# andrew-sha/CUDAFluidSimulator

Measured on AMD Instinct MI355X. Metric: particle-steps/sec (first 41 of the 100 steps of -m time), higher is better.
Workload: dtype f32

## Files before the change

cudafluidsimulator_amd/csrc/sph_api.hip:

```cpp
#include "sph_handle.h"

#include <algorithm>
#include <cmath>
#include <cstdio>
#include <cstdlib>
#include <cstring>
#include <vector>

using namespace sph_host;

namespace {

thread_local std::string g_create_error;

float force_cut2(float h) {
    float h2 = h * h;
    float x = h2;
    for (int k = 0; k < 64; ++k) {
        float nx = std::nextafterf(x, INFINITY);
        if (sqrtf(nx) <= h) x = nx;
        else break;
    }
    return x;
}

Knobs read_knobs() {
    Knobs k;
    if (const char *e = getenv("SPH_SLIM_DIV")) k.slimDiv = atoi(e);
    if (const char *e = getenv("SPH_PIPELINE")) k.pipeline = atoi(e) != 0;
    if (const char *e = getenv("SPH_MASK_POOL_WORDS")) k.maskPoolSet = true, k.maskPoolQuads = strtoull(e, nullptr, 10) / 4;
    if (const char *e = getenv("SPH_ZERO_PAIR_FILTER")) k.zeroPairFilter = atoi(e) != 0;
    if (const char *e = getenv("SPH_PREWARM_COPIES")) k.prewarmCopies = atoi(e);
    if (const char *e = getenv("SPH_TILE_CHUNK")) k.tileChunk = atoi(e);
    if (const char *e = getenv("SPH_XCD_ROTATE")) k.xcdRotate = atoi(e);
    if (const char *e = getenv("SPH_STEP_TRACE")) k.stepTrace = atoi(e) != 0;
    if (const char *e = getenv("SPH_READBACK_SDMA")) k.readbackSdma = atoi(e) != 0;
    return k;
}

void fill_params(sph_handle *h) {
    const SphSettings &s = h->settings;
    DevParams &P = h->P;
    P.h = s.h;
    P.h2 = s.h * s.h;
    P.vcoef = s.v_kernel_coeff;
    P.dcoef = s.d_kernel_coeff;
    P.boxDim = s.boxDim;
    P.boxHi = s.boxDim - s.h;
    P.dt = s.timestep;
    P.cut2 = force_cut2(s.h);
    P.D = (int)s.numCellsPerDim;
    P.morton = h->opt.key_order == SPH_KEY_MORTON ? 1 : 0;
    {
        SphSettings ref{};
        sph_default_settings(&ref, s.numParticles, s.randomInit);
        P.slimDiv = (s.h == ref.h && s.v_kernel_coeff == ref.v_kernel_coeff && s.d_kernel_coeff == ref.d_kernel_coeff) ? 1 : 0;
        if (h->knobs.slimDiv == 0) P.slimDiv = 0;
    }
    if (P.morton) {
        int b = 0;
        while ((1 << b) < P.D) ++b;
        P.numCells = 1 << (3 * b);
    } else {
        P.numCells = P.D * P.D * P.D;
    }
}

int init_positions_reference(const SphSettings &s, float *pos) {
    int n = s.numParticles;
    if (s.randomInit) {
        srand(1);
        for (int i = 0; i < n; i++) {
            float x = rand() / (float)RAND_MAX * (s.boxDim - 2.f) + 1.f;
            float y = rand() / (float)RAND_MAX * (s.boxDim - 2.f) + 1.f;
            float z = rand() / (float)RAND_MAX * (s.boxDim - 2.f) + 1.f;
            pos[3 * i + 0] = x;
            pos[3 * i + 1] = y;
            pos[3 * i + 2] = z;
        }
        return n;
    }
    float spacing = 0.9f * s.h;
    int nx = (int)(floor((s.boxDim - 2 * s.h) / spacing) + 1);
    int ny = nx, nz = nx;
    int count = 0;
    for (int x = 0; x < nx && count < n; x++)
        for (int y = 0; y < ny && count < n; y++)
            for (int z = 0; z < nz && count < n; z++) {
                pos[3 * count + 0] = s.h + spacing * x;
                pos[3 * count + 1] = s.h + spacing * y;
                pos[3 * count + 2] = s.h + spacing * z;
                count++;
            }
    return count;
}

void init_positions_dense(const SphSettings &s, float *pos) {
    int n = s.numParticles;
    int nx = (int)ceil(cbrt((double)n));
    while ((long long)nx * nx * nx < n) nx++;
    while (nx > 1 && (long long)(nx - 1) * (nx - 1) * (nx - 1) >= n) nx--;
    float spacing = nx > 1 ? (s.boxDim - 2 * s.h) / (float)(nx - 1) : 0.f;
    int count = 0;
    for (int x = 0; x < nx && count < n; x++)
        for (int y = 0; y < nx && count < n; y++)
            for (int z = 0; z < nx && count < n; z++) {
                pos[3 * count + 0] = s.h + spacing * x;
                pos[3 * count + 1] = s.h + spacing * y;
                pos[3 * count + 2] = s.h + spacing * z;
                count++;
            }
}

int alloc_device(sph_handle *h) {
    const size_t cap = (size_t)(h->cap > 0 ? h->cap : 1);
    h->external = (h->opt.flags & SPH_FLAG_EXTERNAL_STATE) != 0;
    const size_t posCap = h->external ? 1 : cap;
    for (int b = 0; b < 2; ++b) {
        if (!h->external) {
            HIPCHK(h, h->posBuf[b].alloc(cap));
            HIPCHK(h, h->velBuf[b].alloc(cap));
            h->pos4[b] = h->posBuf[b];
            h->vel4[b] = h->velBuf[b];
            HIPCHK(h, hipMemset(h->pos4[b], 0, cap * sizeof(float4)));
            HIPCHK(h, hipMemset(h->vel4[b], 0, cap * sizeof(float4)));
        }
        HIPCHK(h, h->sortKeys[b].alloc(cap));
        HIPCHK(h, h->sortVals[b].alloc(cap));
        h->ws.keys[b] = h->sortKeys[b];
        h->ws.vals[b] = h->sortVals[b];
        if (!(h->opt.flags & SPH_FLAG_MAPPED_POSITIONS)) {
            HIPCHK(h, h->devPosBuf[b].alloc(posCap * 3));
            h->devPos[b] = h->devPosBuf[b];
        }
        HIPCHK(h, hipMemset(h->ws.keys[b], 0, cap * sizeof(uint32_t)));
        HIPCHK(h, hipMemset(h->ws.vals[b], 0, cap * sizeof(uint32_t)));
        HIPCHK(h, h->computeDone[b].create(hipEventDisableTiming));
        HIPCHK(h, h->copyDone[b].create(hipEventDisableTiming));
    }
    h->ws.capacity = (int)cap;
    h->ws.maxBlocks = (int)sph_sort_workspace_blocks((int)cap);
    HIPCHK(h, h->sortBlockHist.alloc((size_t)1024 * (size_t)(h->ws.maxBlocks > 0 ? h->ws.maxBlocks : 1)));
    HIPCHK(h, h->sortDigitTotal.alloc(1024));
    h->ws.blockHist = h->sortBlockHist;
    h->ws.digitTotal = h->sortDigitTotal;
    for (int b = 0; b < 2; ++b) {
        HIPCHK(h, h->cellTable[b].alloc((size_t)h->P.numCells));
        HIPCHK(h, hipMemset(h->cellTable[b], 0, (size_t)h->P.numCells * sizeof(int2)));
    }
    h->cellRange = h->cellTable[0];
    h->aheadEnabled = h->n < (3 << 19);
    if (h->knobs.pipeline >= 0) h->aheadEnabled = h->knobs.pipeline != 0;
    if (h->opt.flags & SPH_FLAG_MAPPED_POSITIONS) {
        HIPCHK(h, h->hostPos.alloc(posCap * 3, hipHostMallocMapped));
        void *dp = nullptr;
        HIPCHK(h, hipHostGetDevicePointer(&dp, h->hostPos, 0));
        h->devPos[0] = h->devPos[1] = static_cast<float *>(dp);
        h->mappedPos = true;
    } else {
        HIPCHK(h, h->hostPos.alloc(posCap * 3));
    }
    memset(h->hostPos, 0, posCap * 3 * sizeof(float));
    if (h->opt.sweep == SPH_SWEEP_LIST) {
        const double ppc = (double)cap / (0.5 * (double)h->P.numCells);
        const double wordsPerLane = 5.0 * (27.0 * ppc / 32.0) + 24.0;
        unsigned long long quads = (unsigned long long)((double)cap * wordsPerLane * 0.5 * 1.25);
        if (quads < (1ull << 20)) quads = 1ull << 20;
        size_t freeB = 0, totalB = 0;
        if (hipMemGetInfo(&freeB, &totalB) == hipSuccess) {
            const unsigned long long lim = (unsigned long long)(0.4 * (double)freeB) / sizeof(uint4);
            if (quads > lim) quads = lim;
        }
        if (h->knobs.maskPoolSet) quads = h->knobs.maskPoolQuads;
        if (quads > 0xFFFFFFF0ull) quads = 0xFFFFFFF0ull;
        h->maskCapacity = quads;
        HIPCHK(h, h->maskPool.alloc((size_t)(quads ? quads : 1) * 4));
        HIPCHK(h, h->pv8.alloc(cap * 2));
        const size_t hdrWords = 2 * ((cap + 63) / 64 + 1);
        HIPCHK(h, h->maskOff.alloc(hdrWords));
        HIPCHK(h, hipMemset(h->maskOff, 0xFF, hdrWords * sizeof(uint32_t)));
        HIPCHK(h, h->noneList.alloc(hdrWords));
        HIPCHK(h, h->maskCursor.alloc(kCursorBytes / sizeof(unsigned long long)));
        HIPCHK(h, hipMemset(h->maskCursor, 0, kCursorBytes));
        HIPCHK(h, h->hitCount.alloc(cap + 64));
// ... 436 lines not shown
```

cudafluidsimulator_amd/csrc/sph_device.h:

```cpp
#pragma once

#include <hip/hip_runtime.h>
#include <stdint.h>

#include "sph_c_api.h"

#define SPH_WAVE 64

#define SPH_MASS 0.02f
#define SPH_GAS_CONSTANT 1.f
#define SPH_REST_DENSITY 1000.f
#define SPH_VISCOSITY 1.f
#define SPH_GRAVITY -9.8f
#define SPH_ELASTICITY 0.5f
#define SPH_EPS_F (1e-4f)
#define SPH_PUSH_STRENGTH (5.f)
#define SPH_BOX_MAX_X (600)
#define SPH_BOX_MIN_X (200)
#define SPH_BOX_MAX_Y (450)
#define SPH_BOX_MIN_Y (150)

struct DevParams {
    float h;
    float h2;
    float vcoef;
    float dcoef;
    float boxDim;
    float boxHi;
    float dt;
    float cut2;
    int D;
    int numCells;
    int morton;
    int slimDiv;
};

__device__ __forceinline__ uint32_t sph_spread3(uint32_t v) {
    v &= 0x3ffu;
    v = (v | (v << 16)) & 0x030000ffu;
    v = (v | (v << 8)) & 0x0300f00fu;
    v = (v | (v << 4)) & 0x030c30c3u;
    v = (v | (v << 2)) & 0x09249249u;
    return v;
}
__device__ __forceinline__ uint32_t sph_cell_key(const DevParams &P, int cx, int cy, int cz) {
    if (P.morton) return sph_spread3((uint32_t)cx) | (sph_spread3((uint32_t)cy) << 1) | (sph_spread3((uint32_t)cz) << 2);
    return (uint32_t)(cx + cy * P.D + cz * P.D * P.D);
}

__device__ __forceinline__ int wave_min_i32(int v) {
#pragma unroll
    for (int off = 32; off > 0; off >>= 1) v = min(v, __shfl_xor(v, off));
    return v;
}
__device__ __forceinline__ int wave_max_i32(int v) {
#pragma unroll
    for (int off = 32; off > 0; off >>= 1) v = max(v, __shfl_xor(v, off));
    return v;
}
__device__ __forceinline__ uint32_t wave_sum_u32(uint32_t v) {
#pragma unroll
    for (int off = 32; off > 0; off >>= 1) v += __shfl_xor(v, off);
    return v;
}


#define SPH_OOB_RECORDS 8
struct SphOobLog {
    uint32_t count;
    struct { int cell[3]; float pos[3]; } rec[SPH_OOB_RECORDS];
};

struct SortWorkspace {
    uint32_t *keys[2];
    uint32_t *vals[2];
    uint32_t *blockHist;
    uint32_t *digitTotal;
    int capacity;
    int maxBlocks;
    SphOobLog *oob;
    const float4 *velSample;
    float4 *vrefOut;
};
size_t sph_sort_workspace_blocks(int n);
int sph_sort_pairs(const SortWorkspace &ws, int n, int bits, hipStream_t s);
int sph_sort_cells(const SortWorkspace &ws, const DevParams &P, const float4 *pos4, int n, int bits,
                   hipStream_t s, int2 *cellRange, int numCells);

struct Thresholds { uint32_t v[8]; };
struct GatherExtras {
    unsigned long long *cursor = nullptr;
    int cursorWords = 0;
    int *bounds = nullptr;
    const float4 *vref = nullptr;
    unsigned long long *calm = nullptr;
    uint32_t *quietAll = nullptr;
    uint32_t *quietClear = nullptr;
    int quietWords = 0;
    Thresholds thr{};
    int nthr = 0;
};
void sph_launch_gather(const float4 *pos_in, const float4 *vel_in,
                       const uint32_t *perm, const uint32_t *sorted_keys,
                       float4 *pos_out, float4 *vel_out, float4 *pv8, int2 *cellRange, int n,
                       hipStream_t s, const GatherExtras &X = GatherExtras());
void sph_launch_lower_bounds(const uint32_t *sorted_keys, int n, Thresholds thr, int nthr,
                             int *bounds_dev, hipStream_t s);
void sph_launch_partition(const DevParams &P, const float4 *pos_in, const float4 *vel_in, float4 *pos_out,
                          float4 *vel_out, Thresholds thr, int nthr, int n, int *tileCount, int *bounds_dev,
                          hipStream_t s);
size_t sph_partition_tiles(int n);
struct SegmentTable {
    const float4 *spos[8];
    const float4 *svel[8];
    int dst[8];
    int prefix[9];
    int n;
};
void sph_launch_copy_segments(const SegmentTable &T, float4 *dpos, float4 *dvel, hipStream_t s);
void sph_launch_click(const DevParams &P, const int2 *cellRange, float4 *vel4,
                      int mx, int my, hipStream_t s, int zlo = 0, int zhi = 1 << 30);

#define SL_POOL_SHARDS 64
#define SL_CURSOR_STRIDE 32

struct SweepArgs {
    const float4 *pos4;
    float4 *vel4;
    const int2 *cellRange;
    const uint32_t *keys;
    float4 *pos_out;
    float4 *vel_out;
    float *host_order_pos;
    float4 *force_out;
    unsigned long long *pairCounter;
    unsigned long long *stampCounter;
    int i_begin, i_end;
    int i_origin;
    int i_begin2, i_end2;
    int nblk1;
    int n_all;
    int patchHalo;
    int tileChunk;
    int tileRotate;
    uint32_t *maskPool;
    uint32_t *maskOff;
    uint32_t *hitCount;
    unsigned long long *maskCursor;
    uint32_t *noneList;
    unsigned long long maskCapacity;
    float4 *pv8;
    uint32_t *quiet;
    const unsigned long long *calm;
    uint32_t *quietAll;
    const uint32_t *quietHalo;
    int rhoToVel4;
    const int *listHead;
    const int *listNext;
};
void sph_launch_halo_quiet(const float4 *pv8, int lo_end, int hi_begin, int n_all, const float4 *vref,
                           const uint32_t *ownedQuiet, uint32_t *haloQuiet, hipStream_t s);
void sph_launch_link_build(const DevParams &P, const float4 *pos4, int *head, int *next, int n,
                           hipStream_t s);
void sph_launch_density_linked(const DevParams &P, const SweepArgs &A, hipStream_t s);
void sph_launch_force_linked(const DevParams &P, const SweepArgs &A, hipStream_t s);
void sph_launch_density_list(const DevParams &P, const SweepArgs &A, int mathMode, hipStream_t s);
void sph_launch_force_list(const DevParams &P, const SweepArgs &A, int mathMode, hipStream_t s);
void sph_launch_patch_halo(const SweepArgs &A, hipStream_t s);
void sph_launch_density(const DevParams &P, const SweepArgs &A, int mathMode,
                        int sweep, hipStream_t s);
void sph_launch_force(const DevParams &P, const SweepArgs &A, int mathMode,
                      int sweep, hipStream_t s);

struct RenderParams {
    int width, height;
    float Wf, Hf;
    int radius;
    int shade;
};
void sph_launch_render_edges(const RenderParams &R, uint32_t *edge, hipStream_t s);
void sph_launch_render(const RenderParams &R, const float4 *pos4, int n, bool plain, uint32_t *depth, uint32_t *count,
                       const uint32_t *edge, uint32_t *rgb, hipStream_t s);
void sph_launch_render_field(const RenderParams &R, const float4 *pos4, const float4 *vel4, int n, bool plain, int field,
                            bool autoRange, float lo, float hi, unsigned long long *packed, uint32_t *depth, uint32_t *count,
                            const uint32_t *edge, uint32_t *range, uint32_t *rgb, hipStream_t s);

__device__ __forceinline__ uint32_t field_bits(const float4 v, int field) {
    float s;
    if (field == SPH_FIELD_SPEED) s = sqrtf((v.x * v.x + v.y * v.y) + v.z * v.z);
    else if (field == SPH_FIELD_DENSITY) s = v.w;
    else s = fmaxf(0.f, SPH_GAS_CONSTANT * (v.w - SPH_REST_DENSITY));
    return __float_as_uint(s);
}

struct SampleArgs {
    int nx, ny, nz;
    float ox, oy, oz;
    float sx, sy, sz;
    int field;
    const float4 *pos;
    const float4 *vel;
    int stride;
    const int2 *cellRange;
    int n;
};
void sph_launch_sample(const DevParams &P, const SampleArgs &A, bool plain, float *out, hipStream_t s);

struct SurfaceArgs {
    int nx, ny, nz;
    float ox, oy, oz;
    float sx, sy, sz;
    float iso;
};
struct SurfaceBuffers {
    const float *field;
    uint8_t *bits;
    uint32_t *local;
    uint2 *blockSum, *blockOff;
    unsigned long long *totals;
};
int sph_surface_blocks(const SurfaceArgs &A);
void sph_launch_surface_count(const SurfaceArgs &A, bool plain, const SurfaceBuffers &B, hipStream_t s);
void sph_launch_surface_emit(const SurfaceArgs &A, bool plain, const SurfaceBuffers &B, float *verts, uint32_t *tris, hipStream_t s);

struct DiagBlock {
    unsigned long long lo[SPH_DIAG_SUMS];
    long long hi[SPH_DIAG_SUMS];
    unsigned long long saturated;
    uint32_t minKey[SPH_DIAG_EXTREMA];
    uint32_t maxKey[SPH_DIAG_EXTREMA];
    uint32_t range[2];
    uint32_t pad[2];
    unsigned long long hist[SPH_DIAG_BINS];
};
struct DiagArgs {
    const float4 *pos;
    const float4 *vel;
    int stride;
    int n;
    int histField;
    int autoRange;
    float lo, hi;
};
void sph_launch_diagnose(const DiagArgs &A, bool plain, DiagBlock *blk, hipStream_t s);
```

cudafluidsimulator_amd/csrc/sph_handle.h:

```cpp
#pragma once

#include "sph_c_api.h"
#include "sph_device.h"
#include "sph_owned.h"

#include <chrono>
#include <cstdlib>
#include <cstring>
#include <initializer_list>
#include <string>

namespace sph_host {

using sph_owned::DeviceBuf;
using sph_owned::Event;
using sph_owned::PinnedBuf;

struct Knobs {
    int slimDiv = 1;
    int pipeline = -1;
    bool maskPoolSet = false;
    unsigned long long maskPoolQuads = 0;
    bool zeroPairFilter = true;
    int prewarmCopies = 16;
    int tileChunk = -1;
    int xcdRotate = -1;
    bool stepTrace = false;
    bool readbackSdma = true;
};
inline bool plain_path(const char *name) {
    const char *e = getenv(name);
    return e && atoi(e) != 0;
}

constexpr int kEventRing = 64;
constexpr int kCounterWords = 16 + 256 * 16;
constexpr size_t kCursorBytes = (size_t)SL_POOL_SHARDS * SL_CURSOR_STRIDE * sizeof(unsigned long long);

struct PairEvent {
    Event a, b;
    double *target = nullptr;
    bool used = false;
};
constexpr int kPairRing = 48;

struct Outbound {
    Event done, copied;
    bool pending = false;
};
struct OutboundCopy {
    void *dst;
    const void *src;
    size_t bytes;
};

struct StepEvents {
    Event e[6];
    Event c[2];
    bool used = false, hasCopy = false, counted = false;
};

}

struct sph_handle {
    SphSettings settings{};
    SphOptions opt{};
    sph_host::Knobs knobs{};
    DevParams P{};
    int n = 0, cap = 0, device = 0;
    hipStream_t compute = nullptr, copy = nullptr;
    sph_host::DeviceBuf<float4> posBuf[2], velBuf[2];
    float4 *pos4[2] = {nullptr, nullptr};
    float4 *vel4[2] = {nullptr, nullptr};
    int cur = 0;
    int sorted = -1;
    sph_host::DeviceBuf<uint32_t> sortKeys[2], sortVals[2], sortBlockHist, sortDigitTotal;
    SortWorkspace ws{};
    int sortedKeyBuf = 0;
    int2 *cellRange = nullptr;
    sph_host::DeviceBuf<int2> cellTable[2];
    int cellCur = 0;
    sph_host::DeviceBuf<float> devPosBuf[2];
    float *devPos[2] = {nullptr, nullptr};
    sph_host::PinnedBuf<float> hostPos;
    bool hostPosIsInit = false;
    sph_host::PinnedBuf<float4> stage[2];
    sph_host::Event stageFree[2];
    bool mappedPos = false;
    sph_host::DeviceBuf<float4> force4;
    sph_host::DeviceBuf<unsigned long long> pairCounter;
    sph_host::PinnedBuf<unsigned long long> pairHost;
    SphKernelTimes kt{};
    sph_host::DeviceBuf<float4> pv8;
    sph_host::DeviceBuf<uint32_t> maskPool, maskOff;
    sph_host::DeviceBuf<uint32_t> noneList;
    sph_host::DeviceBuf<uint32_t> hitCount;
    sph_host::DeviceBuf<uint32_t> quiet;
    sph_host::DeviceBuf<float4> quietVref;
    sph_host::DeviceBuf<unsigned long long> calm;
    sph_host::DeviceBuf<float4> initPos4;
    sph_host::PinnedBuf<SphOobLog> oobHost;
    uint32_t oobSeen = 0;
    int initZLayers = 0;
    uint64_t hitsRecorded = 0;
    sph_host::DeviceBuf<unsigned long long> maskCursor;
    unsigned long long maskCapacity = 0;
    int zLayers = 0;
    bool ready = false;
    bool gridValid = false;
    int phase = 0;
    std::string err;

    bool gridAhead = false;
    int2 *clickTable = nullptr;
    bool clickValid = false;
    bool aheadEnabled = true;
    sph_host::StepEvents *aheadEv = nullptr;
    sph_host::Event computeDone[2], copyDone[2];
    bool copyPending[2] = {false, false};
    bool stepTimed = false;
    int rbDeferredSlot = -1;
    bool cursorClean = false;
    long long stepIndex = 0;
    sph_host::StepEvents ring[sph_host::kEventRing];
    int ringHead = 0;
    sph_host::StepEvents *curEv = nullptr;
    sph_host::PairEvent pairs[sph_host::kPairRing];
    int pairHead = 0;
    double trEnqueue = 0, trSync = 0, trPost = 0, trBetween = 0, trPh[5] = {0, 0, 0, 0, 0};
    long long trSteps = 0;
    std::chrono::steady_clock::time_point trLastReturn{};
    sph_host::Event trBase;

    bool sdmaOk = false;
    uint64_t hsaGpu = 0, hsaCpu = 0;
    uint64_t rbSig[2] = {0, 0};
    bool rbPending[2] = {false, false};
    uint32_t sdmaEngine = 0;
    double hsaTickSeconds = 0;

    int slabOwnedBegin = 0, slabOwnedEnd = 0;
    bool external = false;
    hipStream_t ownCompute = nullptr;
    sph_host::DeviceBuf<int> boundsDev;
    sph_host::PinnedBuf<int> boundsHost;
    sph_host::DeviceBuf<int> partTiles;

    RenderParams rp{};
    sph_host::DeviceBuf<uint32_t> rDepth, rCount, rEdge, rRgb;
    sph_host::PinnedBuf<uint8_t> frameHost;
    sph_host::Outbound frameOut;
    bool frameValid = false;
    double renderSeconds = 0;
    long long renderFrames = 0;
    sph_host::DeviceBuf<unsigned long long> rPacked;
    sph_host::DeviceBuf<uint32_t> rRange;
    sph_host::PinnedBuf<uint32_t> rangeHost;
    bool fieldFrame = false;

    sph_host::DeviceBuf<float> sampleDev;
    sph_host::PinnedBuf<float> sampleHost;
    size_t sampleCap = 0;
    int sampleDim[3] = {0, 0, 0};
    sph_host::Outbound sampleOut;
    bool sampleValid = false;
    double sampleSeconds = 0;
    long long sampleCount = 0;
    long long sampleTileCalls = 0, samplePlainCalls = 0;

    sph_host::DeviceBuf<float> surfField;
    sph_host::DeviceBuf<uint8_t> surfBits;
    sph_host::DeviceBuf<uint32_t> surfLocal;
    sph_host::DeviceBuf<uint2> surfBlockSum, surfBlockOff;
    sph_host::DeviceBuf<unsigned long long> surfTotalsDev;
    sph_host::PinnedBuf<unsigned long long> surfTotalsHost;
    sph_host::Event surfCounted;
// ... 98 lines not shown
```

cudafluidsimulator_amd/csrc/sph_step.hip:

```cpp
#include "sph_handle.h"

#include <chrono>
#include <cstdio>

using namespace sph_host;

namespace sph_host {

void report_oob(sph_handle *h) {
    if (!h || !h->oobHost) return;
    const uint32_t cnt = h->oobHost->count;
    if (cnt == h->oobSeen) return;
    const int D = h->P.D;
    const uint32_t shown = cnt < SPH_OOB_RECORDS ? cnt : SPH_OOB_RECORDS;
    for (uint32_t k = h->oobSeen < shown ? h->oobSeen : shown; k < shown; ++k) {
        const auto &r = h->oobHost->rec[k];
        const char axis[3] = {'x', 'y', 'z'};
        for (int a = 0; a < 3; ++a)
            if (r.cell[a] < 0 || r.cell[a] >= D)
                printf("OOB particle: %c = %d\n(%f, %f, %f)\n", axis[a], r.cell[a], r.pos[0], r.pos[1], r.pos[2]);
    }
    if (cnt > shown) printf("OOB particle: %u positions outside the grid so far (the first %u listed)\n", cnt, shown);
    fflush(stdout);
    h->oobSeen = cnt;
}

int key_bits(const sph_handle *h) {
    int bits = 1;
    while ((1ll << bits) < (long long)h->P.numCells) ++bits;
    return bits;
}

int tile_chunk(const sph_handle *h, int count, int layers) {
    if (h->knobs.tileChunk >= 0) return h->knobs.tileChunk;
    if (layers <= 0) return 0;
    const long long tiles = ((long long)count + 255) / 256;
    return (int)(tiles / (8ll * layers));
}

SweepArgs make_sweep_args(sph_handle *h) {
    SweepArgs A{};
    const int s = h->sorted;
    A.pos4 = h->pos4[s];
    A.vel4 = h->vel4[s];
    A.cellRange = h->cellRange;
    A.keys = h->ws.keys[h->sortedKeyBuf];
    A.pos_out = h->pos4[s ^ 1];
    A.vel_out = h->vel4[s ^ 1];
    A.host_order_pos = nullptr;
    A.force_out = h->force4;
    A.pairCounter = nullptr;
    A.i_begin = 0;
    A.i_end = h->n;
    A.i_origin = 0;
    A.i_begin2 = A.i_end2 = 0;
    A.nblk1 = 0;
    A.patchHalo = 0;
    A.n_all = h->n;
    A.tileChunk = tile_chunk(h, h->n, h->zLayers);
    A.tileRotate = h->knobs.xcdRotate > 0 ? h->knobs.xcdRotate : 0;
    A.maskPool = h->maskPool;
    A.maskOff = h->maskOff;
    A.noneList = h->noneList;
    A.hitCount = h->hitCount;
    A.maskCursor = h->maskCursor;
    A.maskCapacity = h->maskCapacity;
    A.pv8 = h->pv8;
    A.quiet = h->knobs.zeroPairFilter ? h->quiet.get() : nullptr;
    A.calm = h->calm;
    A.quietAll = A.quiet ? reinterpret_cast<uint32_t *>(h->quietVref + 1) : nullptr;
    A.quietHalo = nullptr;
    A.rhoToVel4 = h->external ? 1 : 0;
    A.listHead = reinterpret_cast<const int *>(h->cellRange);
    A.listNext = reinterpret_cast<const int *>(h->ws.vals[0]);
    return A;
}

GatherExtras gather_extras(sph_handle *h) {
    GatherExtras X;
    if (h->maskCursor) {
        X.cursor = h->maskCursor;
        X.cursorWords = (int)(kCursorBytes / sizeof(unsigned long long));
        h->cursorClean = true;
    }
    if (h->quiet && h->knobs.zeroPairFilter) {
        X.vref = h->quietVref;
        X.calm = h->calm;
        X.quietAll = reinterpret_cast<uint32_t *>(h->quietVref + 1);
        if (h->external) {
            X.quietClear = h->quiet;
            X.quietWords = (int)(2 * (((size_t)h->cap + 63) / 64) + 2);
        }
    }
    return X;
}

int resolve_events(sph_handle *h, StepEvents &se) {
    if (!se.used || se.counted) return SPH_OK;
    HIPCHK(h, hipEventSynchronize(se.e[5]));
    float ms[5];
    for (int k = 0; k < 5; ++k) HIPCHK(h, hipEventElapsedTime(&ms[k], se.e[k], se.e[k + 1]));
    h->kt.hash += ms[0] * 1e-3;
    h->kt.sort += ms[1] * 1e-3;
    h->kt.gather += ms[2] * 1e-3;
    h->kt.density += ms[3] * 1e-3;
    h->kt.force += ms[4] * 1e-3;
    if (se.hasCopy) {
        float cms;
        HIPCHK(h, hipEventSynchronize(se.c[1]));
        HIPCHK(h, hipEventElapsedTime(&cms, se.c[0], se.c[1]));
        h->kt.readback += cms * 1e-3;
    }
    h->kt.steps += 1;
    se.counted = true;
    se.used = false;
    if (h->knobs.stepTrace && h->trBase && se.hasCopy) {
        float t0 = 0, t3 = 0, t5 = 0, c0 = 0, c1 = 0;
        if (hipEventElapsedTime(&t0, h->trBase, se.e[0]) == hipSuccess && hipEventElapsedTime(&t3, h->trBase, se.e[3]) == hipSuccess &&
            hipEventElapsedTime(&t5, h->trBase, se.e[5]) == hipSuccess && hipEventElapsedTime(&c0, h->trBase, se.c[0]) == hipSuccess &&
            hipEventElapsedTime(&c1, h->trBase, se.c[1]) == hipSuccess)
            fprintf(stderr, "sph timeline: grid %.3f..%.3f sweeps ..%.3f | copy %.3f..%.3f\n", t0, t3, t5, c0, c1);
        (void)hipGetLastError();
    }
    return SPH_OK;
}

int begin_step_events(sph_handle *h) {
    StepEvents &se = h->ring[h->ringHead];
    if (se.used) {
        int rc = resolve_events(h, se);
        if (rc) return rc;
    }
    se.used = true;
    se.counted = false;
    se.hasCopy = false;
    h->curEv = &se;
    h->ringHead = (h->ringHead + 1) % kEventRing;
    return SPH_OK;
}

int build_grid_ahead(sph_handle *h) {
    int rc;
    if ((rc = begin_step_events(h))) return rc;
    StepEvents *nextEv = h->curEv;
    if ((rc = sph_phase_grid(h))) return rc;
    h->curEv = nullptr;
    h->aheadEv = nextEv;
    h->gridAhead = true;
    return SPH_OK;
}

int resolve_pair(sph_handle *h, PairEvent &pe) {
    if (!pe.used) return SPH_OK;
    float ms = 0.f;
    HIPCHK(h, hipEventSynchronize(pe.b));
    HIPCHK(h, hipEventElapsedTime(&ms, pe.a, pe.b));
    *pe.target += ms * 1e-3;
    pe.used = false;
    return SPH_OK;
}

int pair_begin(sph_handle *h, double *target, PairEvent **out, hipStream_t stream) {
    PairEvent &pe = h->pairs[h->pairHead];
    int rc = resolve_pair(h, pe);
    if (rc) return rc;
    h->pairHead = (h->pairHead + 1) % kPairRing;
    pe.target = target;
    pe.used = true;
    HIPCHK(h, hipEventRecord(pe.a, stream ? stream : h->compute));
    *out = &pe;
    return SPH_OK;
}

int timed_total(sph_handle *h, double *seconds, long long *count, double *secondsOut, int64_t *countOut, int reset) {
    SPH_ON_DEVICE(h);
    for (auto &pe : h->pairs)
        if (pe.used && pe.target == seconds) {
            int rc = resolve_pair(h, pe);
            if (rc) return rc;
        }
    if (secondsOut) *secondsOut = *seconds;
    if (countOut) *countOut = *count;
    if (reset) {
        *seconds = 0;
        *count = 0;
    }
    return SPH_OK;
}

int outbound_fence(sph_handle *h, Outbound &o) {
    if (o.pending) HIPCHK(h, hipStreamWaitEvent(h->compute, o.copied, 0));
    o.pending = false;
    return SPH_OK;
}

int outbound_send(sph_handle *h, Outbound &o, std::initializer_list<OutboundCopy> copies) {
    HIPCHK(h, o.done.create(hipEventDisableTiming));
    HIPCHK(h, o.copied.create(hipEventDisableTiming));
    HIPCHK(h, hipEventRecord(o.done, h->compute));
    HIPCHK(h, hipStreamWaitEvent(h->copy, o.done, 0));
    for (const OutboundCopy &c : copies) HIPCHK(h, hipMemcpyAsync(c.dst, c.src, c.bytes, hipMemcpyDeviceToHost, h->copy));
    HIPCHK(h, hipEventRecord(o.copied, h->copy));
    o.pending = true;
    return SPH_OK;
}

hipError_t outbound_wait(const Outbound &o) { return o.pending ? hipEventSynchronize(o.copied) : hipSuccess; }

int launch_density(sph_handle *h, SweepArgs &A, hipStream_t stream) {
    if (h->opt.flags & SPH_FLAG_COUNT_PAIRS) A.pairCounter = h->pairCounter;
    if (h->maskCursor && !h->cursorClean) HIPCHK(h, hipMemsetAsync(h->maskCursor, 0, kCursorBytes, stream));
    h->cursorClean = false;
    sph_launch_density(h->P, A, h->opt.math_mode, h->opt.sweep, stream);
    return SPH_OK;
}

void drop_grid_ahead(sph_handle *h) {
    if (!h->gridAhead) return;
    h->gridAhead = false;
    if (h->aheadEv) h->aheadEv->used = false;
    h->aheadEv = nullptr;
    h->gridValid = false;
    h->phase = 0;
}

// ... 270 lines not shown
```

cudafluidsimulator_amd/csrc/sweeps_list.hip:

```cpp
#include "sweep_common.h"

#define SL_NONE 0xFFFFFFFFu

#ifndef SL_WINDOW
#define SL_WINDOW 160
#endif
#ifndef SL_K1_THREADS
#define SL_K1_THREADS 64
#endif

#ifndef SL_K1_WAVES
#define SL_K1_WAVES 6
#endif
__device__ __forceinline__ void sl_store_quiet(const SweepArgs &A, int i, bool valid, float rho, int lane) {
    const unsigned long long calm = A.calm[(i - lane) >> 6];
    const float prs = fmaxf(0.f, SPH_GAS_CONSTANT * (rho - SPH_REST_DENSITY));
    const bool q = valid && prs == 0.f && ((calm >> lane) & 1ull);
    const unsigned long long qb = __ballot(q), vb = __ballot(valid);
    if (lane == 0) {
        reinterpret_cast<unsigned long long *>(A.quiet)[(i - lane) >> 6] = qb;
        if (A.quietAll && qb != vb) *A.quietAll = 0u;
    }
}
__device__ __forceinline__ uint32_t sl_quiet_window(const uint32_t *__restrict__ quiet, uint32_t j) {
// ... 172 lines not shown
                            const float4 *p = (k + u < len) ? cur + k : sent;
                            pj[u] = p[u];
                        }
                        trip(pj);
                    }
                } else {
                    for (; __ballot(k < len); k += SW_UNROLL) {
                        float4 pj[SW_UNROLL];
#pragma unroll
                        for (int u = 0; u < SW_UNROLL; ++u) {
                            const bool in = k + u < len;
                            pj[u] = gcur[in ? k + u : 0];
                            pj[u].x = in ? pj[u].x : 1e18f;
                        }
                        trip(pj);
                    }
                }
                if ((k & 31) != 0) {
                    if (SAMECUT) emit((uint32_t)(jsr + (k & ~31)), (~__builtin_bitreverse32(m)) >> (32 - (k & 31)));
                    else emit((uint32_t)(jsr + (k & ~31)), __builtin_bitreverse32(m) >> (32 - (k & 31)));
                }
                __builtin_amdgcn_fence(__ATOMIC_ACQUIRE, "wavefront");
                __builtin_amdgcn_wave_barrier();
            }
        }
    }
    if (ok && valid) {
        if (pending) myq[(size_t)qidx * SPH_WAVE] = make_uint4(pj0, pm0, 0u, 0u);
        else if (qidx < Q) myq[(size_t)qidx * SPH_WAVE] = make_uint4(0u, 0u, 0u, 0u);
    }
    if (valid) {
        rho = fmaxf(rho, SPH_EPS_F);
        if (A.rhoToVel4) A.vel4[i].w = rho;
        A.pv8[2 * (size_t)i + 1].w = rho;
    }
    if (A.quiet) sl_store_quiet(A, i, valid, rho, lane);
    if (A.hitCount && valid) A.hitCount[i] = hcount;
}

#ifndef SL_SORT_SHIFT
#define SL_SORT_SHIFT 3
#endif
#define SL_DEAL_THREADS 256
#define SL_DEAL_ROWS SL_DEAL_THREADS
#define SL_DEAL_WINDOW (SL_DEAL_ROWS + SL_WINDOW - SPH_WAVE)
static_assert(SL_WINDOW >= SPH_WAVE, "the dealt sweep needs the window");

template <bool FAST, bool SLIM>
__global__ __launch_bounds__(SL_DEAL_THREADS) void k_force_dealt(DevParams P, SweepArgs A) {
    __shared__ uint32_t sortBase[128];
    __shared__ uint16_t rowOf[SL_DEAL_ROWS];
    __shared__ float4 win[2 * SL_DEAL_WINDOW];
    const int t = threadIdx.x, lane = t & 63;
    const bool second = (int)blockIdx.x >= A.nblk1;
    const int rb = second ? A.i_begin2 : A.i_begin, re = second ? A.i_end2 : A.i_end;
    const int chunk = A.tileChunk > 0 ? max(A.tileChunk * 256 / SL_DEAL_ROWS, 1) : 0;
    const int group = ((rb - A.i_origin) >> 6) / (SL_DEAL_ROWS / SPH_WAVE) +
                      xcd_tile(second ? (int)blockIdx.x - A.nblk1 : (int)blockIdx.x,
                               second ? (int)gridDim.x - A.nblk1 : A.nblk1, chunk, A.tileRotate);
    const int R0 = A.i_origin + group * SL_DEAL_ROWS;
    const unsigned long long *const quiet64 = reinterpret_cast<const unsigned long long *>(A.quiet);

    unsigned long long qw = 0ull;
    bool inPlace = false;
    if (A.quiet) {
        const int r0 = R0 + (t & ~63);
        const int lo = max(rb - r0, 0), hi = min(re - r0, 64);
        const unsigned long long vm = hi > lo ? ((hi - lo == 64 ? ~0ull : (1ull << (hi - lo)) - 1ull) << lo) : 0ull;
        if (vm) qw = quiet64[r0 >> 6];
        inPlace = __syncthreads_and((qw & vm) == vm) != 0;
    }
    if (!inPlace) {
        for (int b = t; b < 128; b += SL_DEAL_THREADS) sortBase[b] = 0u;
        __syncthreads();
        const int row = R0 + t;
        const bool counted = row >= rb && row < re && !((qw >> lane) & 1ull);
        const uint32_t bucket = min((counted ? A.hitCount[row] : 0u) >> SL_SORT_SHIFT, 127u);
        const uint32_t slot = atomicAdd(&sortBase[bucket], 1u);
        __syncthreads();
        if (t < SPH_WAVE) {
            const uint32_t a = sortBase[2 * t], b = sortBase[2 * t + 1];
            uint32_t incl = a + b;
#pragma unroll
            for (int off = 1; off < SPH_WAVE; off <<= 1) {
                const uint32_t up = __shfl_up(incl, off);
                incl += t >= off ? up : 0u;
            }
            const uint32_t excl = incl - (a + b);
            sortBase[2 * t] = excl;
            sortBase[2 * t + 1] = excl + a;
        }
        __syncthreads();
        rowOf[sortBase[bucket] + slot] = (uint16_t)t;
    }

    const bool allQuiet = A.quietAll && __builtin_amdgcn_readfirstlane(*A.quietAll) != 0u &&
                          (!A.quietHalo || __builtin_amdgcn_readfirstlane(*A.quietHalo) != 0u);
    const int w0 = max(R0 - (SL_WINDOW - SPH_WAVE) / 2, 0);
    int wlen = max(min(SL_DEAL_WINDOW, A.n_all - w0), 0);
    {
        bool wanted = !allQuiet && wlen > 0;
        if (wanted && A.quiet) {
            const int k0 = w0 >> 6, k1 = (w0 + wlen - 1) >> 6;
            wanted = k0 + t <= k1 && quiet64[k0 + t] != ~0ull;
        }
        if (__syncthreads_or(wanted)) {
            for (int k = t; k < 2 * wlen; k += SL_DEAL_THREADS) win[k] = A.pv8[2 * (size_t)w0 + k];
            __syncthreads();
        } else {
            wlen = 0;
        }
    }

    {
        const int i = R0 + (inPlace ? t : (int)rowOf[t]);
        const bool inRange = i >= rb && i < re;
        const int iSafe = inRange ? i : rb;
        float4 pi = A.pv8[2 * (size_t)iSafe];
        const float4 vi = A.pv8[2 * (size_t)iSafe + 1];
        const float prs_i = fmaxf(0.f, SPH_GAS_CONSTANT * (vi.w - SPH_REST_DENSITY));
        const int rel = iSafe - A.i_origin;
        const uint32_t baseq = inRange ? A.maskOff[2 * (size_t)(rel >> 6)] : SL_NONE;
        const int Q = inRange ? (int)A.maskOff[2 * (size_t)(rel >> 6) + 1] : 0;
        const bool valid = inRange && baseq != SL_NONE;
        ForceAcc F = {0.f, 0.f, 0.f};
        if (!allQuiet) {
            const uint4 *const sbase = reinterpret_cast<const uint4 *>(A.maskPool);
            const uint32_t send = valid ? baseq + (uint32_t)Q * SPH_WAVE : 0u;
            uint32_t sidx = valid ? baseq + (uint32_t)(rel & 63) : 0u;
            uint32_t m = 0, mq[2] = {0u, 0u};
            int jb = 0, jq[2] = {0, 0};
            bool live = true;
            const bool qi = A.quiet && valid && ((A.quiet[i >> 5] >> (i & 31)) & 1u);
            auto fetch = [&]() {
                while (sidx < send) {
                    uint4 q = sbase[sidx];
                    sidx = (q.w == 0u) ? send : sidx + SPH_WAVE;
                    if (qi) {
                        q.y &= ~sl_quiet_window(A.quiet, q.x);
                        q.w &= ~sl_quiet_window(A.quiet, q.z);
                    }
                    if (q.y == 0u) {
                        q.x = q.z;
                        q.y = q.w;
                        q.w = 0u;
                    }
                    jq[0] = (int)q.x;
                    mq[0] = q.y;
                    jq[1] = (int)q.z;
                    mq[1] = q.w;
                    if (q.y != 0u) break;
                }
            };
            fetch();
            if (__ballot(mq[0] != 0u)) {
                auto pop = [&]() -> int {
                    if (m == 0) {
                        m = mq[0];
                        jb = jq[0];
                        mq[0] = mq[1];
                        jq[0] = jq[1];
                        mq[1] = 0;
                        if (mq[0] == 0) fetch();
                    }
                    live = (m | mq[0]) != 0;
                    const bool has = m != 0;
                    const int b = has ? __builtin_ctz(m) : 0;
                    m &= m - 1u;
                    return has ? jb + b : iSafe;
                };
                auto body = [&](const float4 &pj, const float4 &vj) {
                    if (FAST) force_pair_fast(P, pi.x, pi.y, pi.z, vi.x, vi.y, vi.z, prs_i, pj, vj, F);
                    else force_pair<SLIM>(P, pi.x, pi.y, pi.z, vi.x, vi.y, vi.z, prs_i, pj, vj, F);
                };
#define SD_UNDEF4(q) asm volatile("" : "=v"(q.x), "=v"(q.y), "=v"(q.z), "=v"(q.w));
#define SD_FETCH(j, p, v)                                                      \
    SD_UNDEF4(p)                                                               \
    SD_UNDEF4(v)                                                               \
    if ((unsigned)((j)-w0) >= (unsigned)wlen) {                                \
        p = A.pv8[2 * (size_t)(j)];                                            \
        v = A.pv8[2 * (size_t)(j) + 1];                                        \
    }
#define SD_USE(j, p, v)                                                        \
    if ((unsigned)((j)-w0) < (unsigned)wlen) {                                 \
        p = win[2 * ((j)-w0)];                                                 \
        v = win[2 * ((j)-w0) + 1];                                             \
    }                                                                          \
    body(p, v);
                float4 p0 = make_float4(0, 0, 0, 0), v0 = p0, p1 = p0, v1 = p0;
                int j0 = pop();
                SD_FETCH(j0, p0, v0)
                int j1 = pop();
                SD_FETCH(j1, p1, v1)
                for (;;) {
                    SD_USE(j0, p0, v0)
                    if (!__ballot(live)) { SD_USE(j1, p1, v1) break; }
                    j0 = pop();
                    SD_FETCH(j0, p0, v0)
                    SD_USE(j1, p1, v1)
                    if (!__ballot(live)) { SD_USE(j0, p0, v0) break; }
                    j1 = pop();
                    SD_FETCH(j1, p1, v1)
                }
#undef SD_FETCH
#undef SD_USE
#undef SD_UNDEF4
            }
        }
        if (valid) {
            float vx = vi.x, vy = vi.y, vz = vi.z;
            integrate_particle(P, pi, vx, vy, vz, F, vi.w);
            store_particle(A, i, pi, vx, vy, vz, vi.w, F);
        }
    }
}

__global__ __launch_bounds__(256) void k_halo_quiet(const float4 *__restrict__ pv8, int lo_end, int hi_begin, int n_all,
                                                    const float4 *__restrict__ vref, const uint32_t *__restrict__ ownedQuiet,
                                                    uint32_t *__restrict__ haloQuiet) {
    if (*ownedQuiet == 0u) return;
    const int t = blockIdx.x * blockDim.x + threadIdx.x;
    if (t >= lo_end + (n_all - hi_begin)) return;
    const int j = t < lo_end ? t : hi_begin + (t - lo_end);
    const float4 v = pv8[2 * (size_t)j + 1], r = *vref;
    const float prs = fmaxf(0.f, SPH_GAS_CONSTANT * (v.w - SPH_REST_DENSITY));
    if (!(prs == 0.f && v.x == r.x && v.y == r.y && v.z == r.z)) *haloQuiet = 0u;
}
void sph_launch_halo_quiet(const float4 *pv8, int lo_end, int hi_begin, int n_all, const float4 *vref,
                           const uint32_t *ownedQuiet, uint32_t *haloQuiet, hipStream_t s) {
    const int rows = lo_end + (n_all - hi_begin);
    if (rows > 0) k_halo_quiet<<<(rows + 255) / 256, 256, 0, s>>>(pv8, lo_end, hi_begin, n_all, vref, ownedQuiet, haloQuiet);
}

__global__ __launch_bounds__(256) void k_count_hits(SweepArgs A) {
    const int i = A.i_begin + blockIdx.x * blockDim.x + threadIdx.x;
    uint32_t n = 0, dropped = 0;
    if (i < A.i_end) {
        const int rel = i - A.i_origin, wv = rel >> 6;
        const uint32_t baseq = A.maskOff[2 * (size_t)wv];
        const int Q = (int)A.maskOff[2 * (size_t)wv + 1];
        if (baseq != SL_NONE) {
            const uint4 *q4 = reinterpret_cast<const uint4 *>(A.maskPool) + baseq + (rel & 63);
            const bool qi = A.quiet && ((A.quiet[i >> 5] >> (i & 31)) & 1u);
            for (int q = 0; q < Q; ++q) {
                const uint4 t = q4[(size_t)q * SPH_WAVE];
                n += (uint32_t)__builtin_popcount(t.y) + (uint32_t)__builtin_popcount(t.w);
                if (qi)
                    dropped += (uint32_t)__builtin_popcount(t.y & sl_quiet_window(A.quiet, t.x)) +
                               (uint32_t)__builtin_popcount(t.w & sl_quiet_window(A.quiet, t.z));
                if (t.w == 0u) break;
            }
        }
    }
    n = wave_sum_u32(n);
    dropped = wave_sum_u32(dropped);
    if ((threadIdx.x & 63) == 0 && n) {
        atomicAdd(A.pairCounter + 16 + (blockIdx.x & 255) * 16 + 15, (unsigned long long)n);
        atomicAdd(A.pairCounter + 16 + (blockIdx.x & 255) * 16 + 14, (unsigned long long)(n - dropped));
    }
}

void sph_launch_density_list(const DevParams &P, const SweepArgs &A, int mathMode, hipStream_t s) {
    int cnt = A.i_end - A.i_begin;
    if (cnt <= 0) return;
    int blocks = (A.i_end - A.i_origin + SL_K1_THREADS - 1) / SL_K1_THREADS;
    const bool same = P.cut2 == P.h2;
    if (mathMode == 1) {
        if (same) k_density_mask_lds<true, true><<<blocks, SL_K1_THREADS, 0, s>>>(P, A);
        else k_density_mask_lds<true, false><<<blocks, SL_K1_THREADS, 0, s>>>(P, A);
    } else {
        if (same) k_density_mask_lds<false, true><<<blocks, SL_K1_THREADS, 0, s>>>(P, A);
        else k_density_mask_lds<false, false><<<blocks, SL_K1_THREADS, 0, s>>>(P, A);
    }
    if (A.pairCounter) k_count_hits<<<(cnt + 255) / 256, 256, 0, s>>>(A);
}

#define SL_FALLBACK_BLOCKS 512
template <bool FAST, bool SLIM>
__global__ __launch_bounds__(SPH_WAVE) void k_force_fallback(DevParams P, SweepArgs A) {
    const unsigned count = (unsigned)A.maskCursor[1];
    for (unsigned idx = blockIdx.x; idx < count; idx += gridDim.x) {
    const int i = A.i_origin + (int)A.noneList[idx] * SPH_WAVE + (int)threadIdx.x;
    const bool mine = (i >= A.i_begin && i < A.i_end) || (i >= A.i_begin2 && i < A.i_end2);
    if (!__ballot(mine)) continue;
    const int iSafe = mine ? i : A.i_begin;
    float4 pi = A.pv8[2 * (size_t)iSafe];
    const float4 vi = A.pv8[2 * (size_t)iSafe + 1];
    const float prs_i = fmaxf(0.f, SPH_GAS_CONSTANT * (vi.w - SPH_REST_DENSITY));
    int3 c = sweep_cell(P, pi.x, pi.y, pi.z);
    int js[9], je[9];
    load_runs(P, A.cellRange, c, mine, js, je);
    ForceAcc F = {0.f, 0.f, 0.f};
#pragma unroll
    for (int r = 0; r < 9; ++r)
        for (int j = js[r]; j < je[r]; ++j) {
            if (FAST) force_pair_fast(P, pi.x, pi.y, pi.z, vi.x, vi.y, vi.z, prs_i, A.pv8[2 * (size_t)j], A.pv8[2 * (size_t)j + 1], F);
            else force_pair<SLIM>(P, pi.x, pi.y, pi.z, vi.x, vi.y, vi.z, prs_i, A.pv8[2 * (size_t)j], A.pv8[2 * (size_t)j + 1], F);
        }
    if (mine) {
        float vx = vi.x, vy = vi.y, vz = vi.z;
        integrate_particle(P, pi, vx, vy, vz, F, vi.w);
        store_particle(A, i, pi, vx, vy, vz, vi.w, F);
    }
    }
}

__global__ void k_patch_pv8(const float4 *__restrict__ vel4, float4 *__restrict__ pv8, int i_begin,
                            int i_end, int n_all) {
    int t = blockIdx.x * blockDim.x + threadIdx.x;
    int j = t < i_begin ? t : i_end + (t - i_begin);
    if (j < n_all) pv8[2 * (size_t)j + 1] = vel4[j];
}

void sph_launch_patch_halo(const SweepArgs &A, hipStream_t s) {
    const int halo = A.i_begin + (A.n_all - A.i_end);
    if (halo > 0) k_patch_pv8<<<(halo + 255) / 256, 256, 0, s>>>(A.vel4, A.pv8, A.i_begin, A.i_end, A.n_all);
}

void sph_launch_force_list(const DevParams &P, const SweepArgs &A, int mathMode, hipStream_t s) {
    SweepArgs B = A;
    if (B.i_end2 <= B.i_begin2) B.i_begin2 = B.i_end2 = 0;
    if (B.i_end <= B.i_begin) {
        B.i_begin = B.i_begin2;
        B.i_end = B.i_end2;
        B.i_begin2 = B.i_end2 = 0;
    }
    if (B.i_end <= B.i_begin) return;
    if (B.patchHalo) sph_launch_patch_halo(B, s);
    const int wpb = SL_DEAL_ROWS / SPH_WAVE, threads = SL_DEAL_THREADS;
    auto blocks_of = [&](int a, int b) {
        if (b <= a) return 0;
        const int w0 = (a - B.i_origin) >> 6, w1 = (b - B.i_origin + 63) >> 6;
        return (w1 + wpb - 1) / wpb - w0 / wpb;
    };
    B.nblk1 = blocks_of(B.i_begin, B.i_end);
    const int fblocks = B.nblk1 + blocks_of(B.i_begin2, B.i_end2);
    const int blocks = SL_FALLBACK_BLOCKS;
    if (mathMode == 1) {
        k_force_dealt<true, true><<<fblocks, threads, 0, s>>>(P, B);
        k_force_fallback<true, true><<<blocks, SPH_WAVE, 0, s>>>(P, B);
    } else if (P.slimDiv) {
        k_force_dealt<false, true><<<fblocks, threads, 0, s>>>(P, B);
        k_force_fallback<false, true><<<blocks, SPH_WAVE, 0, s>>>(P, B);
    } else {
        k_force_dealt<false, false><<<fblocks, threads, 0, s>>>(P, B);
        k_force_fallback<false, false><<<blocks, SPH_WAVE, 0, s>>>(P, B);
    }
}
```

Baseline: 4.507 billion.

## Software-pipeline force list sweep with inline-asm prefetch of neighbor records and mask quads

Adds a new force-sweep path, enabled by default through a knob, that hand-schedules global loads with inline assembly. Neighbor position/velocity gathers and the next mask-list quad are issued under explicit exec masks, with s_waitcnt vmcnt(2), so two gathers plus a lookahead stay in flight while the previous pair is computed. Position loads are trimmed to dwordx3. The aim is to hide the latency of the dependent mask-list fetch and the gathers in the inner loop. The cost is fragile inline asm that bypasses compiler scheduling, hand-counted waitcnts that could be wrong, and extra register pressure.

```diff
diff --git a/cudafluidsimulator_amd/csrc/sph_api.hip b/cudafluidsimulator_amd/csrc/sph_api.hip
--- a/cudafluidsimulator_amd/csrc/sph_api.hip
+++ b/cudafluidsimulator_amd/csrc/sph_api.hip
@@ -30,6 +30,7 @@
     if (const char *e = getenv("SPH_PIPELINE")) k.pipeline = atoi(e) != 0;
     if (const char *e = getenv("SPH_MASK_POOL_WORDS")) k.maskPoolSet = true, k.maskPoolQuads = strtoull(e, nullptr, 10) / 4;
     if (const char *e = getenv("SPH_ZERO_PAIR_FILTER")) k.zeroPairFilter = atoi(e) != 0;
+    if (const char *e = getenv("SPH_FORCE_PIPELINE")) k.forcePipeline = atoi(e) != 0;
     if (const char *e = getenv("SPH_PREWARM_COPIES")) k.prewarmCopies = atoi(e);
     if (const char *e = getenv("SPH_TILE_CHUNK")) k.tileChunk = atoi(e);
     if (const char *e = getenv("SPH_XCD_ROTATE")) k.xcdRotate = atoi(e);
diff --git a/cudafluidsimulator_amd/csrc/sph_device.h b/cudafluidsimulator_amd/csrc/sph_device.h
--- a/cudafluidsimulator_amd/csrc/sph_device.h
+++ b/cudafluidsimulator_amd/csrc/sph_device.h
@@ -157,6 +157,7 @@
     int rhoToVel4;
     const int *listHead;
     const int *listNext;
+    int forcePipeline;
 };
 void sph_launch_halo_quiet(const float4 *pv8, int lo_end, int hi_begin, int n_all, const float4 *vref,
                            const uint32_t *ownedQuiet, uint32_t *haloQuiet, hipStream_t s);
diff --git a/cudafluidsimulator_amd/csrc/sph_handle.h b/cudafluidsimulator_amd/csrc/sph_handle.h
--- a/cudafluidsimulator_amd/csrc/sph_handle.h
+++ b/cudafluidsimulator_amd/csrc/sph_handle.h
@@ -22,6 +22,7 @@
     bool maskPoolSet = false;
     unsigned long long maskPoolQuads = 0;
     bool zeroPairFilter = true;
+    bool forcePipeline = true;
     int prewarmCopies = 16;
     int tileChunk = -1;
     int xcdRotate = -1;
diff --git a/cudafluidsimulator_amd/csrc/sph_step.hip b/cudafluidsimulator_amd/csrc/sph_step.hip
--- a/cudafluidsimulator_amd/csrc/sph_step.hip
+++ b/cudafluidsimulator_amd/csrc/sph_step.hip
@@ -71,6 +71,7 @@
     A.quietAll = A.quiet ? reinterpret_cast<uint32_t *>(h->quietVref + 1) : nullptr;
     A.quietHalo = nullptr;
     A.rhoToVel4 = h->external ? 1 : 0;
+    A.forcePipeline = h->knobs.forcePipeline ? 1 : 0;
     A.listHead = reinterpret_cast<const int *>(h->cellRange);
     A.listNext = reinterpret_cast<const int *>(h->ws.vals[0]);
     return A;
diff --git a/cudafluidsimulator_amd/csrc/sweeps_list.hip b/cudafluidsimulator_amd/csrc/sweeps_list.hip
--- a/cudafluidsimulator_amd/csrc/sweeps_list.hip
+++ b/cudafluidsimulator_amd/csrc/sweeps_list.hip
@@ -348,6 +348,116 @@
                     if (q.y != 0u) break;
                 }
             };
+            auto body = [&](const float4 &pj, const float4 &vj) {
+                if (FAST) force_pair_fast(P, pi.x, pi.y, pi.z, vi.x, vi.y, vi.z, prs_i, pj, vj, F);
+                else force_pair<SLIM>(P, pi.x, pi.y, pi.z, vi.x, vi.y, vi.z, prs_i, pj, vj, F);
+            };
+            if (A.forcePipeline && !__ballot(qi)) {
+                const uint32_t first = baseq + (uint32_t)(rel & 63);
+                const bool hasS = valid && Q > 0;
+                const unsigned long long hs = __ballot(hasS);
+                if (hs) {
+                    const uint32_t anyq = __builtin_amdgcn_readlane(first, __builtin_ctzll(hs));
+                    const uint32_t lastq = hasS ? first + (uint32_t)(Q - 1) * SPH_WAVE : anyq;
+                    uint32_t la = hasS ? first : SL_NONE;
+                    typedef uint32_t sp_u4 __attribute__((ext_vector_type(4)));
+                    sp_u4 nq;
+                    {
+                        const uint4 q = sbase[min(la, lastq)];
+                        nq = sp_u4{q.x, q.y, q.z, q.w};
+                    }
+                    if (__ballot(la != SL_NONE && nq.y != 0u)) {
+                        uint32_t m2 = 0;
+                        int j2 = 0;
+                        bool took = false;
+                        auto pop = [&]() -> int {
+                            const uint32_t mc = m, m2c = m2, lac = la;
+                            const int jbc = jb, j2c = j2;
+                            const bool need = mc == 0u, take = need && m2c == 0u, ended = lac == SL_NONE;
+                            const uint32_t qx = nq.x, qy = ended ? 0u : nq.y, qz = nq.z, qw = ended ? 0u : nq.w;
+                            const uint32_t mn = need ? (take ? qy : m2c) : mc;
+                            jb = need ? (take ? (int)qx : j2c) : jbc;
+                            m2 = need ? (take ? qw : 0u) : m2c;
+                            j2 = take ? (int)qz : j2c;
+                            const uint32_t lan = (qw == 0u || lac == lastq) ? SL_NONE : lac + SPH_WAVE;
+                            la = take ? lan : lac;
+                            took = take;
+                            live = mn != 0u;
+                            const int b = live ? __builtin_ctz(mn) : 0;
+                            m = mn & (mn - 1u);
+                            return live ? jb + b : iSafe;
+                        };
+#define SP_WAIT(n) asm volatile("s_waitcnt vmcnt(" #n ")");
+#define SP_LANDED_REC(p, v) asm volatile("" : "+v"(p), "+v"(v));
+#define SP_LANDED_QUAD(q) asm volatile("" : "+v"(q));
+#define SP_LOOKAHEAD(mask)                                                                        \
+    {                                                                                             \
+        const uint4 *const a_ = sbase + min(la, lastq);                                           \
+        unsigned long long x_;                                                                    \
+        asm volatile("s_and_saveexec_b64 %1, %3\n\tglobal_load_dwordx4 %0, %2, off\n\ts_mov_b64 exec, %1" \
+                     : "+v"(nq), "=&s"(x_)                                                        \
+                     : "v"(a_), "s"(mask));                                                       \
+    }
+#define SP_GATHER(j, p, v)                                                                        \
+    {                                                                                             \
+        const unsigned long long o_ = __ballot((unsigned)((j)-w0) >= (unsigned)wlen);             \
+        const float4 *const a_ = A.pv8 + 2 * (size_t)(j);                                         \
+        unsigned long long x_;                                                                    \
+        asm volatile("s_and_saveexec_b64 %2, %4\n\tglobal_load_dwordx3 %0, %3, off\n\t"          \
+                     "global_load_dwordx4 %1, %3, off offset:16\n\ts_mov_b64 exec, %2"            \
+                     : "=&v"(p), "=&v"(v), "=&s"(x_)                                              \
+                     : "v"(a_), "s"(o_));                                                         \
+    }
+#define SP_USE(j, p, v)                                                                           \
+    if ((unsigned)((j)-w0) < (unsigned)wlen) {                                                    \
+        const float4 a_ = win[2 * ((j)-w0)], b_ = win[2 * ((j)-w0) + 1];                          \
+        p = sp_f3{a_.x, a_.y, a_.z};                                                              \
+        v = sp_f4{b_.x, b_.y, b_.z, b_.w};                                                        \
+    }                                                                                             \
+    body(make_float4(p.x, p.y, p.z, 0.f), make_float4(v.x, v.y, v.z, v.w));                       \
+    asm volatile("" : "+v"(F.fx), "+v"(F.fy), "+v"(F.fz));
+                        typedef float sp_f3 __attribute__((ext_vector_type(3)));
+                        typedef float sp_f4 __attribute__((ext_vector_type(4)));
+                        sp_f3 p0 = {0.f, 0.f, 0.f}, p1 = p0;
+                        sp_f4 v0 = {0.f, 0.f, 0.f, 0.f}, v1 = v0;
+                        int j0 = pop();
+                        unsigned long long tm = __ballot(took);
+                        SP_GATHER(j0, p0, v0)
+                        int j1 = pop();
+                        tm |= __ballot(took);
+                        SP_LOOKAHEAD(tm)
+                        SP_GATHER(j1, p1, v1)
+                        bool liveA;
+                        do {
+                            SP_WAIT(2)
+                            SP_LANDED_REC(p0, v0)
+                            SP_LANDED_QUAD(nq)
+                            SP_USE(j0, p0, v0)
+                            j0 = pop();
+                            liveA = live;
+                            tm = __ballot(took);
+                            SP_GATHER(j0, p0, v0)
+                            SP_WAIT(2)
+                            SP_LANDED_REC(p1, v1)
+                            SP_USE(j1, p1, v1)
+                            j1 = pop();
+                            tm |= __ballot(took);
+                            SP_LOOKAHEAD(tm)
+                            SP_GATHER(j1, p1, v1)
+                        } while (__ballot(liveA));
+                        SP_WAIT(0)
+                        SP_LANDED_REC(p0, v0)
+                        SP_LANDED_REC(p1, v1)
+                        SP_LANDED_QUAD(nq)
+#undef SP_WAIT
+#undef SP_LANDED_REC
+#undef SP_LANDED_QUAD
+#undef SP_LOOKAHEAD
+#undef SP_GATHER
+#undef SP_USE
+                    }
+                }
+            } else {
             fetch();
             if (__ballot(mq[0] != 0u)) {
                 auto pop = [&]() -> int {
@@ -364,10 +474,6 @@
                     const int b = has ? __builtin_ctz(m) : 0;
                     m &= m - 1u;
                     return has ? jb + b : iSafe;
-                };
-                auto body = [&](const float4 &pj, const float4 &vj) {
-                    if (FAST) force_pair_fast(P, pi.x, pi.y, pi.z, vi.x, vi.y, vi.z, prs_i, pj, vj, F);
-                    else force_pair<SLIM>(P, pi.x, pi.y, pi.z, vi.x, vi.y, vi.z, prs_i, pj, vj, F);
                 };
 #define SD_UNDEF4(q) asm volatile("" : "=v"(q.x), "=v"(q.y), "=v"(q.z), "=v"(q.w));
 #define SD_FETCH(j, p, v)                                                      \
@@ -402,6 +508,7 @@
 #undef SD_USE
 #undef SD_UNDEF4
             }
+            }
         }
         if (valid) {
             float vx = vi.x, vy = vi.y, vz = vi.z;
```

Result: no change. 4.507 billion (median of 4 runs) (+0.0%).
